# hasindu2008/sigtk

Hardware: NVIDIA B200
Metric: event_detection_throughput (higher is better)
Workload: dtype f64

## Files before the change

sigtk_b200/csrc/walk_core.cuh:

```cuda
#pragma once
#include <float.h>
#include <math.h>
#include <stdint.h>
#include <string.h>

#if defined(__CUDACC__)
#define SGW_HD __host__ __device__ __forceinline__
#else
#define SGW_HD inline
#endif

namespace sgpu {
namespace walk {

#if defined(__CUDA_ARCH__)
SGW_HD double dadd(double a, double b) { return __dadd_rn(a, b); }
SGW_HD double dsub(double a, double b) { return __dsub_rn(a, b); }
SGW_HD double dmul(double a, double b) { return __dmul_rn(a, b); }
SGW_HD double dfma(double a, double b, double c) { return __fma_rn(a, b, c); }
SGW_HD double ddiv(double a, double b) { return __ddiv_rn(a, b); }
SGW_HD double dsqrt(double a) { return __dsqrt_rn(a); }
SGW_HD float fadd(float a, float b) { return __fadd_rn(a, b); }
SGW_HD float fsub(float a, float b) { return __fsub_rn(a, b); }
SGW_HD float fmul(float a, float b) { return __fmul_rn(a, b); }
SGW_HD float ffma(float a, float b, float c) { return __fmaf_rn(a, b, c); }
SGW_HD float fdiv(float a, float b) { return __fdiv_rn(a, b); }
SGW_HD float d2f(double a) { return __double2float_rn(a); }
SGW_HD uint32_t d_hi(double a) { return (uint32_t)__double2hiint(a); }
SGW_HD uint32_t d_lo(double a) { return (uint32_t)__double2loint(a); }
SGW_HD uint32_t f_bits(float a) { return __float_as_uint(a); }
SGW_HD float bits_f(uint32_t b) { return __uint_as_float(b); }
SGW_HD float rsqrt_seed(float a) {
    float y;
    asm("rsqrt.approx.ftz.f32 %0, %1;" : "=f"(y) : "f"(a));
    return y;
}
SGW_HD double widen_pos(float a) {
    return __longlong_as_double((long long)((unsigned long long)__float_as_uint(a) * 0x20000000ull + 0x3800000000000000ull));
}
SGW_HD double widen_abs(float a) { return (double)fabsf(a); }
SGW_HD uint32_t shr_clamp(uint32_t x, int s) {
    uint32_t r;
    asm("shr.b32 %0, %1, %2;" : "=r"(r) : "r"(x), "r"(s));
    return r;
}
struct F2 { float lo, hi; };
SGW_HD F2 f2mul(F2 a, F2 b) {
    F2 r;
    asm("{\n\t.reg .b64 a, b, d;\n\tmov.b64 a, {%2, %3};\n\tmov.b64 b, {%4, %5};\n\tmul.rn.f32x2 d, a, b;\n\t"
        "mov.b64 {%0, %1}, d;\n\t}" : "=f"(r.lo), "=f"(r.hi) : "f"(a.lo), "f"(a.hi), "f"(b.lo), "f"(b.hi));
    return r;
}
SGW_HD F2 f2sq(F2 a) {
    F2 r;
    asm("{\n\t.reg .b64 a, d;\n\tmov.b64 a, {%2, %3};\n\tmul.rn.f32x2 d, a, a;\n\tmov.b64 {%0, %1}, d;\n\t}"
        : "=f"(r.lo), "=f"(r.hi) : "f"(a.lo), "f"(a.hi));
    return r;
}
SGW_HD F2 f2add(F2 a, F2 b) {
    F2 r;
    asm("{\n\t.reg .b64 a, b, d;\n\tmov.b64 a, {%2, %3};\n\tmov.b64 b, {%4, %5};\n\tadd.rn.f32x2 d, a, b;\n\t"
        "mov.b64 {%0, %1}, d;\n\t}" : "=f"(r.lo), "=f"(r.hi) : "f"(a.lo), "f"(a.hi), "f"(b.lo), "f"(b.hi));
    return r;
}
SGW_HD F2 f2sub(F2 a, F2 b) {
    F2 r;
    asm("{\n\t.reg .b64 a, b, d;\n\tmov.b64 a, {%2, %3};\n\tmov.b64 b, {%4, %5};\n\tsub.rn.f32x2 d, a, b;\n\t"
        "mov.b64 {%0, %1}, d;\n\t}" : "=f"(r.lo), "=f"(r.hi) : "f"(a.lo), "f"(a.hi), "f"(b.lo), "f"(b.hi));
    return r;
}
SGW_HD F2 f2fma(F2 a, F2 b, F2 c) {
    F2 r;
    asm("{\n\t.reg .b64 a, b, c, d;\n\tmov.b64 a, {%2, %3};\n\tmov.b64 b, {%4, %5};\n\tmov.b64 c, {%6, %7};\n\t"
        "fma.rn.f32x2 d, a, b, c;\n\tmov.b64 {%0, %1}, d;\n\t}"
        : "=f"(r.lo), "=f"(r.hi) : "f"(a.lo), "f"(a.hi), "f"(b.lo), "f"(b.hi), "f"(c.lo), "f"(c.hi));
    return r;
}
#else
SGW_HD double dadd(double a, double b) { return a + b; }
SGW_HD double dsub(double a, double b) { return a - b; }
SGW_HD double dmul(double a, double b) { return a * b; }
SGW_HD double dfma(double a, double b, double c) { return fma(a, b, c); }
SGW_HD double ddiv(double a, double b) { return a / b; }
SGW_HD double dsqrt(double a) { return sqrt(a); }
SGW_HD float fadd(float a, float b) { return a + b; }
SGW_HD float fsub(float a, float b) { return a - b; }
SGW_HD float fmul(float a, float b) { return a * b; }
SGW_HD float ffma(float a, float b, float c) { return fmaf(a, b, c); }
SGW_HD float fdiv(float a, float b) { return a / b; }
SGW_HD float d2f(double a) { return (float)a; }
SGW_HD uint32_t d_hi(double a) { uint64_t b; memcpy(&b, &a, 8); return (uint32_t)(b >> 32); }
SGW_HD uint32_t d_lo(double a) { uint64_t b; memcpy(&b, &a, 8); return (uint32_t)b; }
SGW_HD uint32_t f_bits(float a) { uint32_t b; memcpy(&b, &a, 4); return b; }
SGW_HD float bits_f(uint32_t b) { float a; memcpy(&a, &b, 4); return a; }
SGW_HD float rsqrt_seed(float a) { return (float)(1.0 / sqrt((double)a)); }
SGW_HD double widen_pos(float a) {
    uint32_t b; memcpy(&b, &a, 4);
    const uint64_t v = (uint64_t)b * 0x20000000ull + 0x3800000000000000ull;
    double r; memcpy(&r, &v, 8); return r;
}
SGW_HD double widen_abs(float a) { return (double)fabsf(a); }
SGW_HD uint32_t shr_clamp(uint32_t x, int s) { return (unsigned)s < 32u ? x >> s : 0u; }
struct F2 { float lo, hi; };
SGW_HD F2 f2mul(F2 a, F2 b) { F2 r; r.lo = a.lo * b.lo; r.hi = a.hi * b.hi; return r; }
SGW_HD F2 f2sq(F2 a) { F2 r; r.lo = a.lo * a.lo; r.hi = a.hi * a.hi; return r; }
SGW_HD F2 f2add(F2 a, F2 b) { F2 r; r.lo = a.lo + b.lo; r.hi = a.hi + b.hi; return r; }
SGW_HD F2 f2sub(F2 a, F2 b) { F2 r; r.lo = a.lo - b.lo; r.hi = a.hi - b.hi; return r; }
SGW_HD F2 f2fma(F2 a, F2 b, F2 c) { F2 r; r.lo = fmaf(a.lo, b.lo, c.lo); r.hi = fmaf(a.hi, b.hi, c.hi); return r; }
#endif

template <int RNA>
struct Cfg {
    static constexpr int w1 = RNA ? 7 : 3;
    static constexpr int w2 = 2 * w1;
    static constexpr int LAG = w2 - 1;
    static constexpr int R1 = RNA ? 8 : 4;
    static constexpr int R2 = RNA ? 16 : 8;
    static constexpr int U = RNA ? 16 : 8;
    static constexpr int FILL = 2;
    static_assert(FILL * U >= 2 * w2 - 1, "fill covers the look-back of the first step");
};
template <int RNA> SGW_HD float thr_short() { return RNA ? 2.5f : 1.4f; }
template <int RNA> SGW_HD float thr_long() { return 9.0f; }
template <int RNA> SGW_HD float peak_h() { return RNA ? 1.0f : 0.2f; }

template <int W>
SGW_HD double ddivw(double a) {
    constexpr double r = 1.0 / (double)W;
    const double q0 = dmul(a, r);
    const double e = dfma(-(double)W, q0, a);
    return dfma(e, r, q0);
}
template <int W>
SGW_HD float fdivw(float a) {
    constexpr float r = 1.0f / (float)W;
    const float q0 = fmul(a, r);
    const float e = ffma(-(float)W, q0, a);
    return ffma(e, r, q0);
}

template <int WA, int WB>
SGW_HD F2 fdivw2(F2 a) {
    const F2 r = {1.0f / (float)WA, 1.0f / (float)WB};
    const F2 nw = {-(float)WA, -(float)WB};
    const F2 q0 = f2mul(a, r);
    const F2 e = f2fma(nw, q0, a);
    return f2fma(e, r, q0);
}

SGW_HD float tail(float delta, float scaled, float scaled_half, float cv, bool& ok) {
    const double ch = widen_pos(scaled_half);
    const double y0 = widen_pos(rsqrt_seed(scaled));
    const double th = dmul(ch, y0);
    const double eh = dfma(-th, y0, 0.5);
    const double q0 = dmul(widen_abs(delta), y0);
    const double q = dfma(q0, eh, q0);
    ok = ok & ((d_lo(q) * 8u - ((0x10000000u - 1024u) << 3)) >= (2048u << 3)) & (cv >= 2.0e-29f);
    return d2f(q);
}

template <int W>
SGW_HD void window_terms(double D, double E, float& A, double& Lq, float& B, double& Vd, double& B2d) {
    A = d2f(ddivw<W>(D));
    const F2 de = {d2f(D), d2f(E)};
    const F2 bv = fdivw2<W, W>(de);
    Lq = dsub(ddivw<W>(E), widen_pos(fmul(A, A)));
    B = bv.lo;
    Vd = widen_pos(bv.hi);
    B2d = widen_pos(fmul(B, B));
}
template <int W>
SGW_HD void tstat_two(float A0, double L0, float B0, double V0, double B0sq, float A1, double L1, float B1, double V1,
                      double B1sq, float& t0, bool& ok0, float& t1, bool& ok1) {
    const double acc0 = dsub(dadd(L0, V0), B0sq);
    const double acc1 = dsub(dadd(L1, V1), B1sq);
    const F2 cv = {d2f(acc0), d2f(acc1)};
    const F2 sc = fdivw2<W, W>(cv);
    const F2 half = {0.5f, 0.5f};
    const F2 sh = f2mul(sc, half);
#if defined(WALK_X_NOTAIL)
    t0 = fmul(fsub(B0, A0), sc.lo); t1 = fmul(fsub(B1, A1), sh.hi);
#else
    t0 = tail(fsub(B0, A0), sc.lo, sh.lo, cv.lo, ok0);
    t1 = tail(fsub(B1, A1), sc.hi, sh.hi, cv.hi, ok1);
#endif
}

template <class Io>
SGW_HD float sample_pa(const Io& io, int i, int n, float off, float unit) {
    if (i < 0 || i >= n) return 0.0f;
    int v[4];
    io.load8(i & ~7, v);
    const int q = i & 7;
    const int word = q < 2 ? v[0] : q < 4 ? v[1] : q < 6 ? v[2] : v[3];
    const int raw = (q & 1) ? (word >> 16) : (int)(int16_t)(word & 0xffff);
    return fmul(fadd((float)raw, off), unit);
}
template <class Io>
SGW_HD void window_sums(const Io& io, int a, int w, int n, float off, float unit, double& S, double& Q) {
    S = 0.0; Q = 0.0;
    for (int i = a; i < a + w; i++) {
        const float x = sample_pa(io, i, n, off, unit);
        S = dadd(S, (double)x);
        Q = dadd(Q, (double)fmul(x, x));
    }
}
SGW_HD float tstat_from_sums(double sum1, double ssq1, double sum2d, double ssq2d, int w) {
    const float wf = (float)w;
    const float sum2 = d2f(sum2d), ssq2 = d2f(ssq2d);
    const float mean1 = d2f(ddiv(sum1, (double)wf));
    const float mean2 = fdiv(sum2, wf);
    double acc = ddiv(ssq1, (double)wf);
    acc = dsub(acc, (double)fmul(mean1, mean1));
    acc = dadd(acc, (double)fdiv(ssq2, wf));
    acc = dsub(acc, (double)fmul(mean2, mean2));
    const float cv = fmaxf(d2f(acc), FLT_MIN);
    const float delta = fsub(mean2, mean1);
    return d2f(ddiv(fabs((double)delta), dsqrt((double)fdiv(cv, wf))));
}
template <class Io>
SGW_HD float tstat_exact(const Io& io, int i, int w, int n, float off, float unit) {
    double sum1, ssq1, sum2d, ssq2d;
    window_sums(io, i - w, w, n, off, unit, sum1, ssq1);
    window_sums(io, i, w, n, off, unit, sum2d, ssq2d);
    return tstat_from_sums(sum1, ssq1, sum2d, ssq2d, w);
}
template <class Io>
struct SlidingT {
    double s1, q1, s2, q2;
    int at;
    SGW_HD SlidingT() : s1(0.0), q1(0.0), s2(0.0), q2(0.0), at(-1) {}
    SGW_HD float next(const Io& io, int i, int w, int n, float off, float unit) {
        if (!(i >= w && i + w <= n)) { at = -1; return 0.0f; }
        if (at != i - 1) {
            window_sums(io, i - w, w, n, off, unit, s1, q1);
            window_sums(io, i, w, n, off, unit, s2, q2);
        } else {
            const float xa = sample_pa(io, i - 1 - w, n, off, unit);
            const float xb = sample_pa(io, i - 1, n, off, unit);
            const float xc = sample_pa(io, i - 1 + w, n, off, unit);
            const double da = (double)xa, db = (double)xb, dc = (double)xc;
            const double qa = (double)fmul(xa, xa), qb = (double)fmul(xb, xb), qc = (double)fmul(xc, xc);
            s1 = dadd(dsub(s1, da), db); q1 = dadd(dsub(q1, qa), qb);
            s2 = dadd(dsub(s2, db), dc); q2 = dadd(dsub(q2, qb), qc);
        }
        at = i;
        return tstat_from_sums(s1, q1, s2, q2, w);
    }
};
constexpr int PS_NONE = 0x7fff0000;
constexpr int PS_OPEN = 0x40000000;
constexpr int LS_PRED = -0x40000000;
constexpr int LS_CONT = 0x7fffffff;
struct WalkDet {
    float s_pv; int s_ps;
    int l_start;
    bool l_hot;
};
SGW_HD void det_cold(WalkDet& d, int first_step) {
    d.s_pv = FLT_MAX; d.s_ps = PS_NONE;
    d.l_start = first_step; d.l_hot = false;
}

struct Canon { int v[8]; };
template <int RNA>
SGW_HD Canon canon_of(const WalkDet& d, int b) {
    Canon c;
    (void)b;
    c.v[0] = (int)f_bits(d.s_pv); c.v[1] = d.s_ps; c.v[2] = 0; c.v[3] = 0; c.v[4] = 0; c.v[5] = 0;
    c.v[6] = d.l_start; c.v[7] = 0;
    return c;
}

template <int RNA> struct PkCfg {
    static constexpr int LEAD = 32 - Cfg<RNA>::U;
#if defined(WALK_TEST_FAR)
    static constexpr int FAR = 0;
#else
    static constexpr int FAR = LEAD - (Cfg<RNA>::w1 / 2 + 1);
#endif
};
struct PeakAcc { uint32_t mk; int oldest; int jobs, job_ls, job_end; };
struct NoEmit { SGW_HD void operator()(int) const {} };

template <bool SHORT, int RNA, class E>
SGW_HD int det_one(float& pv, int& ps, int m, int u, float c, float thr, PeakAcc& acc, bool& big2, int& p2,
                   const E& on_emit) {
    constexpr int w = SHORT ? Cfg<RNA>::w1 : Cfg<RNA>::w2;
    const float h = peak_h<RNA>();
    const bool none = ps == PS_NONE;
    const float df = fsub(c, pv);
    const float pvm = none ? fminf(pv, c) : fmaxf(pv, c);
    const bool rise1 = none & (df > h);
    const bool gt2 = !none & (df > 0.0f);
    big2 = !none & (pvm > thr);
    const bool drop = big2 & (df < -h);
    p2 = gt2 ? ((ps & PS_OPEN) | u) : ps;
    const int p3 = drop ? (p2 & ~PS_OPEN) : p2;
    const int over = (u - (w / 2 + 1)) - p3;
    const bool emit = over >= 0;
    acc.mk |= shr_clamp(1u << (PkCfg<RNA>::LEAD + m - (w / 2 + 1)), over);
    if (emit) on_emit(p3);
    pv = (rise1 | emit) ? c : pvm;
    ps = emit ? PS_NONE : p3;
    ps = rise1 ? (u | PS_OPEN) : ps;
    return over;
}

struct DualDet {
    float s_pv; int s_ps;
    float l_pv; int l_ps; int l_mt;
};
SGW_HD void dual_cold(DualDet& d, int first_step) {
    d.s_pv = FLT_MAX; d.s_ps = PS_NONE;
    d.l_pv = FLT_MAX; d.l_ps = PS_NONE; d.l_mt = first_step - 1;
}
SGW_HD Canon dual_canon(const DualDet& d, int b) {
    Canon c;
    c.v[0] = (int)f_bits(d.s_pv); c.v[1] = d.s_ps; c.v[2] = (int)f_bits(d.l_pv); c.v[3] = d.l_ps;
    c.v[4] = d.l_mt >= b ? d.l_mt : -1;
    c.v[5] = 0; c.v[6] = 0; c.v[7] = 0;
    return c;
}
template <int RNA, class E>
SGW_HD void dual_step(DualDet& d, int u, float c1, float c2, const E& on_emit) {
    bool maskl, unused_b; int p2, unused_p;
    PeakAcc unused; unused.mk = 0u; unused.oldest = 0;
    det_one<true, RNA>(d.s_pv, d.s_ps, 0, u, c1, thr_short<RNA>(), unused, maskl, p2, on_emit);
    d.l_mt = maskl ? (p2 & ~PS_OPEN) + Cfg<RNA>::w1 : d.l_mt;
    d.l_ps = maskl ? PS_NONE : d.l_ps;
    d.l_pv = maskl ? FLT_MAX : d.l_pv;
    const float c2m = d.l_mt < u ? c2 : FLT_MAX;
    det_one<false, RNA>(d.l_pv, d.l_ps, 0, u, c2m, thr_long<RNA>(), unused, unused_b, unused_p, on_emit);
}

constexpr int ZMAX = 1023;
struct LongK {
    float c0;
    float ca;
    float cw;
    float h2;
    float t2w;
    float cB;
    float thr;
};
template <int RNA>
SGW_HD LongK long_consts(int c0, float off, float thr_long) {
    constexpr float w = (float)Cfg<RNA>::w2;
    const float u = 5.9604644775390625e-08f;
    LongK k;
    k.c0 = (float)c0;
    const float M = fmul(fadd(fabsf(fadd(k.c0, off)), (float)(ZMAX + 2)), 1.0001f);
    k.ca = fmul(fmul(8.0f * u * w, M), 1.0001f);
    k.cw = w * (1.0f + 0.000244140625f);
    k.thr = thr_long;
    const float thr2 = fmul(thr_long, thr_long);
    k.h2 = fmul(thr2, 0.5f);
    k.t2w = fmul(thr2, w);
    k.cB = fmul(fmul(fmul(thr2, 64.0f * u * w * w), fmul(M, M)), 1.0001f);
    return k;
}
SGW_HD bool long_candidate(float dS, float T, float Q, const LongK& k) {
    const float g = fadd(fabsf(dS), k.ca);
    const float sq = ffma(T, T, fmul(dS, dS));
    const float lhs = ffma(fmul(g, g), k.cw, ffma(sq, k.h2, k.cB));
    const float rhs = fmul(Q, k.t2w);
    return !(lhs < rhs);
}

constexpr int DIRTY_BLOCKS = 3;
static_assert(2 * Cfg<0>::w2 - 1 <= 2 * Cfg<0>::U + 0 && 2 * Cfg<1>::w2 - 1 <= 2 * Cfg<1>::U, "windows reach at most two blocks ahead");

template <int RNA>
struct Rings {
    using C = Cfg<RNA>;
    double P[C::R1], PQ[C::R1];
    float A1[C::R1];
    double L1[C::R1];
    float T1c[C::w1];
    static constexpr int ZH2 = 2 * C::w2 - C::U;
    float Z1[C::U], Z2[ZH2];
    float zdS, zT, zQ;
    SGW_HD void clear() {
#pragma unroll
        for (int k = 0; k < C::R1; k++) { P[k] = 0.0; PQ[k] = 0.0; A1[k] = 0.0f; L1[k] = 0.0; }
#pragma unroll
        for (int k = 0; k < C::w1; k++) T1c[k] = 0.0f;
#pragma unroll
        for (int k = 0; k < C::U; k++) Z1[k] = 0.0f;
#pragma unroll
        for (int k = 0; k < ZH2; k++) Z2[k] = 0.0f;
        zdS = 0.0f; zT = 0.0f; zQ = 0.0f;
    }
};

template <int RNA, bool DIRECT, class E, class Io>
SGW_HD void det_step(WalkDet& d, int m, int u, float c1, bool cand, bool rec, PeakAcc& acc, const E& on_emit, Io& io) {
    bool maskl; int p2;
    const int over = det_one<true, RNA>(d.s_pv, d.s_ps, m, u, c1, thr_short<RNA>(), acc, maskl, p2, on_emit);
    acc.oldest = acc.oldest > over ? acc.oldest : over;
    bool hot = d.l_hot;
    if (maskl & hot & rec) {
        if (DIRECT) io.job(d.l_start, u);
        else { acc.job_ls = d.l_start; acc.job_end = u; acc.jobs++; }
    }
    const int ls = (p2 & ~PS_OPEN) + Cfg<RNA>::w1 + 1;
    d.l_start = maskl ? (ls > u ? ls : u) : d.l_start;
    hot = (hot & !maskl) | ((u >= d.l_start) & cand);
    d.l_hot = hot;
}

template <int RNA> struct Redo { WalkDet d; PeakAcc acc; float t1c[Cfg<RNA>::w1]; };
template <int RNA, bool EDGE, class Io>
#if defined(__CUDACC__)
__host__ __device__ __noinline__
#else
inline
#endif
Redo<RNA> redo_block(Io& io, Redo<RNA> in, int tau0, int n, int sh, bool rec, float off, float unit, float thr_long) {
    using C = Cfg<RNA>;
    constexpr int w1 = C::w1, w2 = C::w2, U = C::U;
    (void)thr_long;
    float e1[U];
    SlidingT<Io> slide;
    for (int m = 0; m < U; m++) e1[m] = slide.next(io, tau0 + m - w1 + 1, w1, n, off, unit);
    Redo<RNA> r;
    r.d = in.d; r.acc.mk = 0u; r.acc.oldest = 0; r.acc.jobs = 0;
    const int u0 = tau0 - w2 + 1 + sh;
    for (int m = 0; m < U; m++) {
        const int j2 = tau0 + m - w2 + 1;
        const float c1 = m >= w1 ? e1[m - w1] : in.t1c[m];
        if (!EDGE || (j2 >= 1 && j2 < n)) {
            PeakAcc unused; unused.mk = 0u; unused.oldest = 0; unused.jobs = 0;
            det_step<RNA, true>(r.d, 0, u0 + m, c1, true, rec, unused, [&](int pos) { if (rec) io.peak(pos); }, io);
        }
    }
    for (int k = 0; k < w1; k++) r.t1c[k] = e1[U - w1 + k];
    return r;
}

template <int RNA, bool EDGE, class Io>
SGW_HD void walk_block(Rings<RNA>& g, WalkDet& d, const float (&x)[Cfg<RNA>::U], const float (&z)[Cfg<RNA>::U], int tau0,
                       int n, int sh, bool rec, bool live, bool live_t1, int dirty, int zdirty, float off, float unit,
                       const LongK& lk, Io& io) {
    using C = Cfg<RNA>;
    constexpr int w1 = C::w1, w2 = C::w2, M1 = C::R1 - 1, M2 = C::R2 - 1, U = C::U;
    float t1v[U];
    bool ok = true, ok_t1 = true;
    const WalkDet d0 = d;
    PeakAcc acc;
    acc.mk = 0u; acc.oldest = 0; acc.jobs = 0;
    const int u0 = tau0 - w2 + 1 + sh;
    float xq[U];
#pragma unroll
    for (int m = 0; m < U; m += 2) {
        const F2 p = {x[m], x[m + 1]};
        const F2 q = f2sq(p);
        xq[m] = q.lo; xq[m + 1] = q.hi;
    }
    float zdS = g.zdS, zT = g.zT, zQ = g.zQ;
#pragma unroll
    for (int m0 = 0; m0 < U; m0 += 2) {
        float a1[2], b1[2]; double l1[2], v1[2], b1sq[2];
        float al[2]; double ll[2];
#pragma unroll
        for (int h = 0; h < 2; h++) {
            const int m = m0 + h;
            const double xd = widen_pos(x[m]);
            const double qd = widen_pos(xq[m]);
            const double pn = dadd(g.P[m & M1], EDGE ? (x[m] > 0.0f ? xd : 0.0) : xd);
            const double pqn = dadd(g.PQ[m & M1], EDGE ? (x[m] > 0.0f ? qd : 0.0) : qd);
            g.P[(m + 1) & M1] = pn;
            g.PQ[(m + 1) & M1] = pqn;
            const int s1 = (m - w1 + 1) & M1;
            const int s1l = (m - 2 * w1 + 1) & M1;
            const double d1 = dsub(pn, g.P[s1]), e1 = dsub(pqn, g.PQ[s1]);
            window_terms<w1>(d1, e1, a1[h], l1[h], b1[h], v1[h], b1sq[h]);
            al[h] = g.A1[s1l]; ll[h] = g.L1[s1l];
        }
        bool k0 = true, k1 = true;
        tstat_two<w1>(al[0], ll[0], b1[0], v1[0], b1sq[0], al[1], ll[1], b1[1], v1[1], b1sq[1], t1v[m0], k0, t1v[m0 + 1], k1);
#pragma unroll
        for (int h = 0; h < 2; h++) {
            const int m = m0 + h;
            bool kh = h ? k1 : k0;
            const int j1 = tau0 + m - w1 + 1;
            if (EDGE) {
                const bool in1 = (j1 >= w1) & (j1 + w1 <= n);
                kh = kh | !in1;
                t1v[m] = in1 ? t1v[m] : 0.0f;
            }
            if (m >= U - w1) ok_t1 = ok_t1 & kh; else ok = ok & kh;
            const int s1 = (m - w1 + 1) & M1;
            g.A1[s1] = a1[h]; g.L1[s1] = l1[h];
        }
#pragma unroll
        for (int h = 0; h < 2; h++) {
            const int m = m0 + h;
            const float zn = z[m];
            const float zm = m >= w2 ? z[m >= w2 ? m - w2 : 0] : g.Z1[m < w2 ? m + U - w2 : 0];
            const float zo = m >= 2 * w2 - U ? g.Z1[m >= 2 * w2 - U ? m + U - 2 * w2 : 0] : g.Z2[m < 2 * w2 - U ? m : 0];
#if defined(WALK_X_NOCAND)
            zT = fadd(zT, zn); (void)zm; (void)zo;
            bool cand = false;
#else
            zT = fadd(zT, fsub(zn, zo));
            zQ = fadd(zQ, fsub(fmul(zn, zn), fmul(zo, zo)));
            zdS = fadd(fadd(zdS, fadd(zn, zo)), fmul(zm, -2.0f));
            bool cand = long_candidate(zdS, zT, zQ, lk);
#endif
            const int j2 = tau0 + m - w2 + 1;
            if (EDGE) cand = cand & (j2 >= w2) & (j2 + w2 <= n);
            cand = cand | (zdirty > 0);
            const float c1 = m >= w1 ? t1v[m >= w1 ? m - w1 : 0] : g.T1c[m < w1 ? m : 0];
#if defined(WALK_X_NODET)
            d.s_pv = fadd(d.s_pv, c1); d.l_hot = d.l_hot | cand;
#elif defined(WALK_X_NOLIFE)
            { bool mk_; int p2_; const int over_ = det_one<true, RNA>(d.s_pv, d.s_ps, m, u0 + m, c1, thr_short<RNA>(), acc, mk_, p2_, NoEmit());
              acc.oldest = acc.oldest > over_ ? acc.oldest : over_; d.l_hot = d.l_hot | (cand & mk_); d.l_start += p2_ & 1; }
#else
            if (!EDGE || (j2 >= 1 && j2 < n)) det_step<RNA, false>(d, m, u0 + m, c1, cand, rec, acc, NoEmit(), io);
#endif
        }
    }
    g.zdS = zdS; g.zT = zT; g.zQ = zQ;
#pragma unroll
    for (int k = 0; k < Rings<RNA>::ZH2; k++) g.Z2[k] = g.Z1[k + U - Rings<RNA>::ZH2];
#pragma unroll
    for (int k = 0; k < U; k++) g.Z1[k] = z[k];
#if defined(WALK_TEST_REDO)
    ok = ok & ((tau0 / U) % 3 != 0);
#endif
    if (dirty > 0) { ok = false; ok_t1 = false; }
    if ((!ok & live) | (!ok_t1 & live_t1) | (rec & ((acc.oldest > PkCfg<RNA>::FAR) | (acc.jobs > 1)))) {
        Redo<RNA> in;
        in.d = d0; in.acc = acc;
#pragma unroll
        for (int k = 0; k < w1; k++) in.t1c[k] = g.T1c[k];
        const Redo<RNA> r = redo_block<RNA, EDGE>(io, in, tau0, n, sh, rec, off, unit, lk.thr);
        d = r.d; acc = r.acc;
#pragma unroll
        for (int k = 0; k < w1; k++) t1v[U - w1 + k] = r.t1c[k];
    }
    if (rec && acc.mk) io.peaks32(u0 - PkCfg<RNA>::LEAD, acc.mk);
    if (acc.jobs == 1) io.job(acc.job_ls, acc.job_end);
#pragma unroll
    for (int k = 0; k < w1; k++) g.T1c[k] = t1v[U - w1 + k];
}

SGW_HD uint32_t n_chunks(uint32_t n, uint32_t L) { return (n + L - 1u) / L; }

SGW_HD void cvt8(const int (&v)[4], float off, float unit, float c0, float* x, float* z) {
    const F2 bias = {8421376.0f, 8421376.0f}, off2 = {off, off}, unit2 = {unit, unit}, c2 = {c0, c0};
#pragma unroll
    for (int k = 0; k < 4; k++) {
        const uint32_t w = (uint32_t)v[k] ^ 0x80008000u;
        F2 r;
        r.lo = bits_f(0x4b000000u | (w & 0xffffu));
        r.hi = bits_f(0x4b000000u | (w >> 16));
        r = f2sub(r, bias);
        const F2 zz = f2sub(r, c2);
        r = f2mul(f2add(r, off2), unit2);
        x[2 * k] = r.lo;
        x[2 * k + 1] = r.hi;
        z[2 * k] = zz.lo;
        z[2 * k + 1] = zz.hi;
    }
}
SGW_HD void cvt8(const int (&v)[4], float off, float unit, float* x) {
    const F2 bias = {8421376.0f, 8421376.0f}, off2 = {off, off}, unit2 = {unit, unit};
#pragma unroll
    for (int k = 0; k < 4; k++) {
        const uint32_t w = (uint32_t)v[k] ^ 0x80008000u;
        F2 r;
        r.lo = bits_f(0x4b000000u | (w & 0xffffu));
        r.hi = bits_f(0x4b000000u | (w >> 16));
        r = f2mul(f2add(f2sub(r, bias), off2), unit2);
        x[2 * k] = r.lo;
        x[2 * k + 1] = r.hi;
    }
}
#if defined(__CUDA_ARCH__)
SGW_HD uint32_t min_s16x2(uint32_t a, uint32_t b) { return __vmins2(a, b); }
SGW_HD uint32_t max_s16x2(uint32_t a, uint32_t b) { return __vmaxs2(a, b); }
#else
SGW_HD uint32_t min_s16x2(uint32_t a, uint32_t b) {
    const int16_t al = (int16_t)(a & 0xffff), ah = (int16_t)(a >> 16), bl = (int16_t)(b & 0xffff), bh = (int16_t)(b >> 16);
    return (uint32_t)(uint16_t)(al < bl ? al : bl) | ((uint32_t)(uint16_t)(ah < bh ? ah : bh) << 16);
}
SGW_HD uint32_t max_s16x2(uint32_t a, uint32_t b) {
    const int16_t al = (int16_t)(a & 0xffff), ah = (int16_t)(a >> 16), bl = (int16_t)(b & 0xffff), bh = (int16_t)(b >> 16);
    return (uint32_t)(uint16_t)(al > bl ? al : bl) | ((uint32_t)(uint16_t)(ah > bh ? ah : bh) << 16);
}
#endif

#if defined(__CUDA_ARCH__)
SGW_HD bool any_le_s16x2(uint32_t a, uint32_t b) { return __vcmples2(a, b) != 0u; }
#else
SGW_HD bool any_le_s16x2(uint32_t a, uint32_t b) {
    return (int16_t)(a & 0xffff) <= (int16_t)(b & 0xffff) || (int16_t)(a >> 16) <= (int16_t)(b >> 16);
}
#endif
constexpr int LOW_MARGIN = 64;
SGW_HD int low_threshold(float off, bool* can) {
    float tf = floorf(-off);
    tf = tf < -40000.0f ? -40000.0f : tf > 40000.0f ? 40000.0f : tf;
    int t = (int)tf;
    for (int k = 0; k < 4 && fadd((float)(t + 1), off) <= 0.0f; k++) t++;
    for (int k = 0; k < 4 && fadd((float)t, off) > 0.0f; k++) t--;
    t += LOW_MARGIN;
    *can = t >= -32768;
    return t > 32767 ? 32767 : t < -32768 ? -32768 : t;
}
SGW_HD uint32_t pack_s16x2(int t) { return ((uint32_t)t & 0xffffu) * 0x10001u; }
SGW_HD int s16_lo(uint32_t v) { return (int)(int16_t)(v & 0xffffu); }
SGW_HD int s16_hi(uint32_t v) { return (int)v >> 16; }

SGW_HD int pivot_of(int a, int b, int c) {
    const int lo = a < b ? a : b, hi = a < b ? b : a;
    return c < lo ? lo : c > hi ? hi : c;
}

template <class Io>
SGW_HD void zero_low8(Io& io, int t, const int (&v)[4], int low_t, float* x) {
    uint32_t lo = 0xffffffffu, hi = 0u;
#pragma unroll
    for (int q = 0; q < 8; q++) {
        const int raw = (q & 1) ? (v[q >> 1] >> 16) : (int)(int16_t)(v[q >> 1] & 0xffff);
        if (raw <= low_t) {
            const uint32_t a = f_bits(x[q]) & 0x7fffffffu;
            if (a != 0u) { lo = a < lo ? a : lo; hi = a > hi ? a : hi; }
            x[q] = 0.0f;
        }
    }
    io.low_samples(t, lo, hi);
}

struct BlockCvt {
    bool can_low, zlo_on, zhi_on, pa;
    int low_t;
    uint32_t low2, zlo2, zhi2;
};
SGW_HD BlockCvt block_cvt(float off, int c0, bool want_pa) {
    BlockCvt k;
    k.low_t = low_threshold(off, &k.can_low);
    k.low2 = pack_s16x2(k.low_t);
    k.zlo2 = pack_s16x2(c0 - ZMAX - 1 < -32768 ? -32768 : c0 - ZMAX - 1);
    k.zhi2 = pack_s16x2(c0 + ZMAX + 1 > 32767 ? 32767 : c0 + ZMAX + 1);
    k.zlo_on = c0 - ZMAX - 1 >= -32768; k.zhi_on = c0 + ZMAX + 1 <= 32767;
    k.pa = want_pa;
    return k;
}
template <class Io>
SGW_HD void cvt_group(Io& io, const BlockCvt& k, const LongK& lk, const int (&v)[4], int t8, bool own, float off, float unit,
                      float* x, float* z, uint32_t& bmin, uint32_t& bmax, int& dirty) {
    const uint32_t m8 = min_s16x2(min_s16x2((uint32_t)v[0], (uint32_t)v[1]), min_s16x2((uint32_t)v[2], (uint32_t)v[3]));
    bmin = min_s16x2(bmin, m8);
    bmax = max_s16x2(max_s16x2(bmax, (uint32_t)v[0]), max_s16x2((uint32_t)v[1], max_s16x2((uint32_t)v[2], (uint32_t)v[3])));
    cvt8(v, off, unit, lk.c0, x, z);
    if (k.pa && own) io.store_pa8(t8, x);
    if (k.can_low & any_le_s16x2(m8, k.low2)) {
        dirty = DIRTY_BLOCKS;
        zero_low8(io, t8, v, k.low_t, x);
    }
}
template <int U>
SGW_HD void clamp_far(const BlockCvt& k, uint32_t bmin, uint32_t bmax, float* z, int& zdirty) {
    if ((k.zlo_on & any_le_s16x2(bmin, k.zlo2)) | (k.zhi_on & any_le_s16x2(k.zhi2, bmax))) {
        zdirty = DIRTY_BLOCKS;
#pragma unroll
        for (int q = 0; q < U; q++)
            z[q] = z[q] > (float)(ZMAX + 1) ? (float)(ZMAX + 1) : z[q] < -(float)(ZMAX + 1) ? -(float)(ZMAX + 1) : z[q];
    }
}

#if !defined(WALK_PF_BLOCKS)
#define WALK_PF_BLOCKS 12
#endif

template <int RNA, class Io>
SGW_HD void walk_interior(Io& io, int n, float off, float unit, int sh, int L, int W, int k, float thr_long) {
    using C = Cfg<RNA>;
    constexpr int U = C::U;
    const int s0 = k * L, s1 = s0 + L;
    const int t_live = s0 - W;
    Rings<RNA> g;
    g.clear();
    WalkDet d;
    det_cold(d, 0);
    float x[U], z[U];
    int v[4];
    uint32_t vmin = 0x7fff7fffu, vmax = 0x80008000u;
    int dirty = 0, zdirty = 0;
    int vn[U / 8][4];
#pragma unroll
    for (int h = 0; h < U / 8; h++) io.load8(t_live - C::FILL * U + 8 * h, vn[h]);
    const int c0 = pivot_of(s16_lo((uint32_t)vn[0][0]), s16_hi((uint32_t)vn[0][0]), s16_lo((uint32_t)vn[0][1]));
    const LongK lk = long_consts<RNA>(c0, off, thr_long);
    const BlockCvt bc = block_cvt(off, c0, io.want_pa());
#pragma unroll 1
    for (int tau = t_live - C::FILL * U; tau < s1; tau += U) {
        const bool own = tau >= s0;
        if (tau == t_live) det_cold(d, t_live - C::LAG + sh);
        if (tau == s0) {
            io.put_begin(canon_of<RNA>(d, s0 - C::LAG + sh));
            d.l_start = LS_PRED; d.l_hot = false;
        }
        const int tn = tau + U < s1 ? tau + U : tau;
        io.prefetch(tau + WALK_PF_BLOCKS * U < s1 ? tau + WALK_PF_BLOCKS * U : tau);
        uint32_t bmin = 0x7fff7fffu, bmax = 0x80008000u;
#pragma unroll
        for (int h = 0; h < U / 8; h++) {
#pragma unroll
            for (int q = 0; q < 4; q++) v[q] = vn[h][q];
            io.load8(tn + 8 * h, vn[h]);
            cvt_group(io, bc, lk, v, tau + 8 * h, own, off, unit, x + 8 * h, z + 8 * h, bmin, bmax, dirty);
        }
        vmin = min_s16x2(vmin, bmin);
        vmax = max_s16x2(vmax, bmax);
        clamp_far<U>(bc, bmin, bmax, z, zdirty);
        walk_block<RNA, false>(g, d, x, z, tau, n, sh, own, tau >= t_live, tau >= t_live - U, dirty, zdirty, off, unit, lk, io);
        dirty = dirty > 0 ? dirty - 1 : 0;
        zdirty = zdirty > 0 ? zdirty - 1 : 0;
    }
    if (d.l_hot) io.job(d.l_start, LS_CONT);
    io.put_end(canon_of<RNA>(d, s1 - C::LAG + sh));
    const int rmin0 = s16_lo(vmin), rmin1 = s16_hi(vmin);
    const int rmax0 = s16_lo(vmax), rmax1 = s16_hi(vmax);
    io.witness(rmin0 < rmin1 ? rmin0 : rmin1, rmax0 > rmax1 ? rmax0 : rmax1, bc.can_low ? bc.low_t : -32769);
}

#if defined(__CUDACC__)
#define SGW_PHASE __host__ __device__ __noinline__
#else
#define SGW_PHASE inline
#endif
template <int RNA>
struct EdgeCtx {
    Rings<RNA> g;
    WalkDet d;
    int rmin, rmax, dirty, zdirty;
    int n, sh, s0, s1, t_live, last, low_t, c0;
    float off, unit;
    bool pa;
    LongK lk;
    BlockCvt bc;
};
template <int RNA, class Io>
SGW_HD void edge_block_begin(Io& io, EdgeCtx<RNA>& e, int tau) {
    using C = Cfg<RNA>;
    if (e.last && tau == e.t_live) det_cold(e.d, e.t_live - C::LAG + e.sh);
    if (e.last && tau == e.s0) {
        io.put_begin(canon_of<RNA>(e.d, e.s0 - C::LAG + e.sh));
        e.d.l_start = LS_PRED; e.d.l_hot = false;
    }
}
template <int RNA, class Io>
SGW_PHASE void edge_inner(Io& io, EdgeCtx<RNA>& ec, int tau_from, int tau_to) {
    using C = Cfg<RNA>;
    constexpr int U = C::U;
    const int turns = io.warp_max(tau_to > tau_from ? (tau_to - tau_from) / U : 0);
    EdgeCtx<RNA> e = ec;
    float x[U], z[U];
    int vn[U / 8][4];
    if (tau_from < tau_to) {
#pragma unroll
        for (int h = 0; h < U / 8; h++) io.load8(tau_from + 8 * h, vn[h]);
    }
    int tau = tau_from;
#pragma unroll 1
    for (int turn = 0; turn < turns; turn++, tau += U) {
        if (tau >= tau_to) continue;
        const bool own = tau >= e.s0;
        edge_block_begin<RNA>(io, e, tau);
        const int tn = tau + U < tau_to ? tau + U : tau;
        io.prefetch(tau + WALK_PF_BLOCKS * U < tau_to ? tau + WALK_PF_BLOCKS * U : tau);
        uint32_t bmin = 0x7fff7fffu, bmax = 0x80008000u;
#pragma unroll
        for (int h = 0; h < U / 8; h++) {
            int v[4];
#pragma unroll
            for (int q = 0; q < 4; q++) v[q] = vn[h][q];
            io.load8(tn + 8 * h, vn[h]);
            cvt_group(io, e.bc, e.lk, v, tau + 8 * h, own, e.off, e.unit, x + 8 * h, z + 8 * h, bmin, bmax, e.dirty);
        }
        if (own) {
            const int b0 = s16_lo(bmin), b1 = s16_hi(bmin), c0x = s16_lo(bmax), c1x = s16_hi(bmax);
            e.rmin = b0 < e.rmin ? b0 : e.rmin; e.rmin = b1 < e.rmin ? b1 : e.rmin;
            e.rmax = c0x > e.rmax ? c0x : e.rmax; e.rmax = c1x > e.rmax ? c1x : e.rmax;
        }
        clamp_far<U>(e.bc, bmin, bmax, z, e.zdirty);
        walk_block<RNA, false>(e.g, e.d, x, z, tau, e.n, e.sh, own, tau >= e.t_live, tau >= e.t_live - U, e.dirty, e.zdirty,
                               e.off, e.unit, e.lk, io);
        e.dirty = e.dirty > 0 ? e.dirty - 1 : 0;
        e.zdirty = e.zdirty > 0 ? e.zdirty - 1 : 0;
    }
    ec = e;
}
template <int RNA, class Io>
SGW_PHASE void edge_checked(Io& io, EdgeCtx<RNA>& ec, int tau_from, int tau_to) {
    using C = Cfg<RNA>;
    constexpr int U = C::U;
    const int turns = io.warp_max(tau_to > tau_from ? (tau_to - tau_from) / U : 0);
    EdgeCtx<RNA> e = ec;
    float x[U], z[U];
    const int n = e.n, c0 = e.c0, low_t = e.low_t;
    int tau = tau_from;
#pragma unroll 1
    for (int turn = 0; turn < turns; turn++, tau += U) {
        if (tau >= tau_to) continue;
        const bool own = tau >= e.s0;
        edge_block_begin<RNA>(io, e, tau);
#pragma unroll
        for (int h = 0; h < U / 8; h++) {
            const int t8 = tau + 8 * h;
            int v[4] = {0, 0, 0, 0};
            if (t8 < n) io.load8(t8, v);
            float y[8], zy[8];
            cvt8(v, e.off, e.unit, e.lk.c0, y, zy);
#pragma unroll
            for (int q = 0; q < 8; q++) {
                const bool in = t8 + q < n;
                const int raw = (q & 1) ? (v[q >> 1] >> 16) : (int)(int16_t)(v[q >> 1] & 0xffff);
                const bool low = in & (raw <= low_t);
                x[8 * h + q] = (in & !low) ? y[q] : 0.0f;
                const bool zbad = in & ((raw - c0 > ZMAX) | (c0 - raw > ZMAX));
                z[8 * h + q] = !in ? 0.0f : !zbad ? zy[q] : raw > c0 ? (float)(ZMAX + 1) : -(float)(ZMAX + 1);
                if (zbad) e.zdirty = DIRTY_BLOCKS;
                if (low) {
                    e.dirty = DIRTY_BLOCKS;
                    const uint32_t a = f_bits(y[q]) & 0x7fffffffu;
                    io.low_samples(t8 + q, a != 0u ? a : 0xffffffffu, a);
                }
                if (own && in && t8 + q < e.s1) {
                    e.rmin = raw < e.rmin ? raw : e.rmin;
                    e.rmax = raw > e.rmax ? raw : e.rmax;
                    if (e.pa) io.store_pa1(t8 + q, y[q]);
                }
            }
        }
        walk_block<RNA, true>(e.g, e.d, x, z, tau, n, e.sh, own, tau >= e.t_live, tau >= e.t_live - U, e.dirty, e.zdirty,
                              e.off, e.unit, e.lk, io);
        e.dirty = e.dirty > 0 ? e.dirty - 1 : 0;
        e.zdirty = e.zdirty > 0 ? e.zdirty - 1 : 0;
    }
    ec = e;
}

template <int RNA, class Io>
SGW_HD void walk_edge(Io& io, int n, float off, float unit, int sh, int L, int W, int last, float thr_long) {
    using C = Cfg<RNA>;
    constexpr int U = C::U;
    const uint32_t nch = n_chunks((uint32_t)n, (uint32_t)L);
    const bool none = nch == 0u || (last && nch < 2u);
    EdgeCtx<RNA> e;
    e.n = n; e.sh = sh; e.off = off; e.unit = unit; e.last = last;
    e.s0 = last ? (int)(nch - 1u) * L : 0;
    const bool to_end = last || nch == 1u;
    e.s1 = to_end ? n : L;
    e.t_live = last ? e.s0 - W : 0;
    const int step_end = to_end ? n : e.s1 - C::LAG;
    e.g.clear();
    det_cold(e.d, sh + 1);
    e.rmin = 32767; e.rmax = -32768;
    bool can_low;
    const int low_t0 = low_threshold(off, &can_low);
    e.low_t = can_low ? low_t0 : -32769;
    e.dirty = 0; e.zdirty = 0;
    e.pa = io.want_pa();
    const int t_first = last ? e.t_live - C::FILL * U : 0;
    e.c0 = 0;
    if (!none) {
        int v0[4] = {0, 0, 0, 0};
        io.load8(t_first, v0);
        const int a = s16_lo((uint32_t)v0[0]), b = t_first + 1 < n ? s16_hi((uint32_t)v0[0]) : a;
        e.c0 = pivot_of(a, b, t_first + 2 < n ? s16_lo((uint32_t)v0[1]) : a);
    }
    e.lk = long_consts<RNA>(e.c0, off, thr_long);
    e.bc = block_cvt(off, e.c0, e.pa);
    constexpr int INNER_MIN = (2 * C::w2 - 1 + U - 1) / U * U;
    const int tau_end = none ? t_first : (step_end + C::LAG + U - 1) / U * U;
    int in0 = t_first > INNER_MIN ? t_first : INNER_MIN;
    in0 = in0 < tau_end ? in0 : tau_end;
    int in1 = n / U * U;
    in1 = in1 < tau_end ? in1 : tau_end;
    in1 = in1 > in0 ? in1 : in0;
    edge_checked<RNA>(io, e, t_first, in0);
    edge_inner<RNA>(io, e, in0, in1);
    edge_checked<RNA>(io, e, in1, tau_end);
    if (none) return;
    if (to_end) {
        if (e.d.l_hot) io.job(e.d.l_start, n + sh);
    } else {
        if (e.d.l_hot) io.job(e.d.l_start, LS_CONT);
        io.put_end(canon_of<RNA>(e.d, e.s1 - C::LAG + sh));
    }
    if (!last) io.peak(sh);
    if (e.rmin <= e.rmax) io.witness(e.rmin, e.rmax, e.low_t);
}

template <int RNA, class Jo>
SGW_HD void long_job(Jo& io, int n, int sh, float off, float unit, int L, int k, int l_start, int end, float thr_long) {
    using C = Cfg<RNA>;
    constexpr int w1 = C::w1, w2 = C::w2;
    for (int kk = k - 1; l_start == LS_PRED && kk >= 0; kk--) l_start = io.end_lstart(kk);
    if (l_start == LS_PRED) return;
    const int stop = n + sh;
    const int own_end = end == LS_CONT ? (k + 1) * L - C::LAG + sh : (end < stop ? end : stop);
    float pv = FLT_MAX; int ps = PS_NONE;
    PeakAcc unused; unused.mk = 0u; unused.oldest = 0;
    bool b2; int p2;
    SlidingT<Jo> slide;
    int u = l_start;
    for (; u + 4 <= own_end; u += 4) {
        float t[4];
#pragma unroll
        for (int q = 0; q < 4; q++) t[q] = slide.next(io, u + q - sh, w2, n, off, unit);
#pragma unroll
        for (int q = 0; q < 4; q++)
            det_one<false, RNA>(pv, ps, 0, u + q, t[q], thr_long, unused, b2, p2, [&](int pos) { io.peak(pos); });
    }
    for (; u < own_end; u++)
        det_one<false, RNA>(pv, ps, 0, u, slide.next(io, u - sh, w2, n, off, unit), thr_long, unused, b2, p2,
                            [&](int pos) { io.peak(pos); });
    if (end != LS_CONT) return;
    float spv; int sps;
    io.end_short(k, &spv, &sps);
    u = own_end;
    SlidingT<Jo> slide1;
    for (; u < stop; u++) {
        const float t1 = slide1.next(io, u - sh, w1, n, off, unit);
        const float t2 = slide.next(io, u - sh, w2, n, off, unit);
        det_one<true, RNA>(spv, sps, 0, u, t1, thr_short<RNA>(), unused, b2, p2, NoEmit());
        if (b2) return;
        det_one<false, RNA>(pv, ps, 0, u, t2, thr_long, unused, b2, p2, [&](int pos) { io.peak(pos); });
    }
}

}
}
```

Baseline: 127.1.

## Rework long-window candidate test into pairwise FMA form with tighter clamp range

Rewrites the long-window candidate filter as a single sign test of a precomputed quadratic form (k1*dS^2 + T^2 - 2w*Q + K0), evaluated for two consecutive samples at once with paired float ops and shared running-sum updates. It also lowers the clamp range for RNA so the long-window sums stay exact in float, and drops an unused parameter from redo_block. The goal is fewer float instructions per sample in the hot walk loop. The risks are a more conservative bound that flags more candidates and more clamping for RNA inputs, which sends more work to the slow path.

```diff
diff --git a/sigtk_b200/csrc/walk_core.cuh b/sigtk_b200/csrc/walk_core.cuh
--- a/sigtk_b200/csrc/walk_core.cuh
+++ b/sigtk_b200/csrc/walk_core.cuh
@@ -119,6 +119,9 @@
     static constexpr int U = RNA ? 16 : 8;
     static constexpr int FILL = 2;
     static_assert(FILL * U >= 2 * w2 - 1, "fill covers the look-back of the first step");
+    static constexpr int ZFAR = RNA ? 773 : 1023;
+    static_assert(2 * w2 * (ZFAR + 1) * (ZFAR + 1) <= (1 << 24), "long-window sums exact in float");
+    static_assert(w2 % 2 == 0 && U % 2 == 0 && (2 * w2 - U) % 2 == 0, "the long window's pairs sit at even indices");
 };
 template <int RNA> SGW_HD float thr_short() { return RNA ? 2.5f : 1.4f; }
 template <int RNA> SGW_HD float thr_long() { return 9.0f; }
@@ -337,35 +340,40 @@
 constexpr int ZMAX = 1023;
 struct LongK {
     float c0;
-    float ca;
-    float cw;
-    float h2;
-    float t2w;
-    float cB;
+    float k1;
+    float K0;
+    float n2w;
     float thr;
 };
 template <int RNA>
 SGW_HD LongK long_consts(int c0, float off, float thr_long) {
     constexpr float w = (float)Cfg<RNA>::w2;
+    constexpr float cw = 2.0f * w * (1.0f + 0.000244140625f);
     const float u = 5.9604644775390625e-08f;
     LongK k;
     k.c0 = (float)c0;
+    k.thr = thr_long;
+    k.n2w = -2.0f * w;
     const float M = fmul(fadd(fabsf(fadd(k.c0, off)), (float)(ZMAX + 2)), 1.0001f);
-    k.ca = fmul(fmul(8.0f * u * w, M), 1.0001f);
-    k.cw = w * (1.0f + 0.000244140625f);
-    k.thr = thr_long;
+    const float a = fmul(fmul(8.0f * u * w, M), 1.0001f);
     const float thr2 = fmul(thr_long, thr_long);
-    k.h2 = fmul(thr2, 0.5f);
-    k.t2w = fmul(thr2, w);
-    k.cB = fmul(fmul(fmul(thr2, 64.0f * u * w * w), fmul(M, M)), 1.0001f);
+    k.k1 = fmul(fadd(1.0f, fmul(fdiv(fmul(cw, 1.0009765625f), thr2), 1.0001f)), 1.0001f);
+    k.K0 = fmul(fadd(fdiv(fmul(fmul(cw, 1025.0f), fmul(a, a)), thr2), fmul(128.0f * u * w * w, fmul(M, M))), 1.0001f);
+    const bool in_range = (thr_long >= 9.5367431640625e-07f) & (M <= 1.099511627776e12f);
+    k.k1 = in_range ? k.k1 : 0.0f;
+    k.K0 = in_range ? k.K0 : INFINITY;
     return k;
 }
+SGW_HD F2 long_test(F2 dS, F2 T, F2 Q, const LongK& k, float n2w_) {
+    const F2 n2w = {n2w_, n2w_}, k1 = {k.k1, k.k1}, K0 = {k.K0, k.K0};
+    const F2 r1 = f2fma(Q, n2w, K0);
+    const F2 r2 = f2fma(f2mul(k1, dS), dS, r1);
+    return f2fma(T, T, r2);
+}
+SGW_HD bool long_cold(float r) { return (f_bits(r) >> 31) != 0u; }
 SGW_HD bool long_candidate(float dS, float T, float Q, const LongK& k) {
-    const float g = fadd(fabsf(dS), k.ca);
-    const float sq = ffma(T, T, fmul(dS, dS));
-    const float lhs = ffma(fmul(g, g), k.cw, ffma(sq, k.h2, k.cB));
-    const float rhs = fmul(Q, k.t2w);
-    return !(lhs < rhs);
+    const F2 dS2 = {dS, dS}, T2 = {T, T}, Q2 = {Q, Q};
+    return !long_cold(long_test(dS2, T2, Q2, k, k.n2w).lo);
 }
 
 constexpr int DIRTY_BLOCKS = 3;
@@ -417,10 +425,9 @@
 #else
 inline
 #endif
-Redo<RNA> redo_block(Io& io, Redo<RNA> in, int tau0, int n, int sh, bool rec, float off, float unit, float thr_long) {
+Redo<RNA> redo_block(Io& io, Redo<RNA> in, int tau0, int n, int sh, bool rec, float off, float unit) {
     using C = Cfg<RNA>;
     constexpr int w1 = C::w1, w2 = C::w2, U = C::U;
-    (void)thr_long;
     float e1[U];
     SlidingT<Io> slide;
     for (int m = 0; m < U; m++) e1[m] = slide.next(io, tau0 + m - w1 + 1, w1, n, off, unit);
@@ -494,31 +501,43 @@
             const int s1 = (m - w1 + 1) & M1;
             g.A1[s1] = a1[h]; g.L1[s1] = l1[h];
         }
+        uint32_t lr[2];
+        {
+            const int b1 = m0 >= w2 ? m0 - w2 : m0 + U - w2, b2 = m0 >= 2 * w2 - U ? m0 + U - 2 * w2 : m0;
+            const F2 zn = {z[m0], z[m0 + 1]};
+            const F2 zm = m0 >= w2 ? F2{z[b1], z[b1 + 1]} : F2{g.Z1[b1], g.Z1[b1 + 1]};
+            const F2 zo = m0 >= 2 * w2 - U ? F2{g.Z1[b2], g.Z1[b2 + 1]} : F2{g.Z2[b2], g.Z2[b2 + 1]};
+#if defined(WALK_X_NOCAND)
+            zT = fadd(zT, fadd(zn.lo, zn.hi)); (void)zm; (void)zo;
+            lr[0] = 0xffffffffu; lr[1] = 0xffffffffu;
+#else
+            const F2 sp = f2add(zn, zo);
+            const F2 dz = f2sub(zn, zo);
+            const F2 m2 = {-2.0f, -2.0f};
+            const F2 ds = f2fma(zm, m2, sp);
+            F2 S, T, Q;
+            T.lo = fadd(zT, dz.lo);
+            T.hi = fadd(T.lo, dz.hi);
+            S.lo = fadd(zdS, ds.lo);
+            S.hi = fadd(S.lo, ds.hi);
+            Q.lo = ffma(dz.lo, sp.lo, zQ);
+            Q.hi = ffma(dz.hi, sp.hi, Q.lo);
+            zT = T.hi; zdS = S.hi; zQ = Q.hi;
+            const F2 r = long_test(S, T, Q, lk, -2.0f * w2);
+            lr[0] = f_bits(r.lo); lr[1] = f_bits(r.hi);
+#endif
+        }
 #pragma unroll
         for (int h = 0; h < 2; h++) {
             const int m = m0 + h;
-            const float zn = z[m];
-            const float zm = m >= w2 ? z[m >= w2 ? m - w2 : 0] : g.Z1[m < w2 ? m + U - w2 : 0];
-            const float zo = m >= 2 * w2 - U ? g.Z1[m >= 2 * w2 - U ? m + U - 2 * w2 : 0] : g.Z2[m < 2 * w2 - U ? m : 0];
-#if defined(WALK_X_NOCAND)
-            zT = fadd(zT, zn); (void)zm; (void)zo;
-            bool cand = false;
+            const int j2 = tau0 + m - w2 + 1;
+            const float c1 = m >= w1 ? t1v[m >= w1 ? m - w1 : 0] : g.T1c[m < w1 ? m : 0];
+#if defined(WALK_X_NODET)
+            d.s_pv = fadd(d.s_pv, c1); d.l_hot = d.l_hot | ((lr[h] >> 31) == 0u);
 #else
-            zT = fadd(zT, fsub(zn, zo));
-            zQ = fadd(zQ, fsub(fmul(zn, zn), fmul(zo, zo)));
-            zdS = fadd(fadd(zdS, fadd(zn, zo)), fmul(zm, -2.0f));
-            bool cand = long_candidate(zdS, zT, zQ, lk);
-#endif
-            const int j2 = tau0 + m - w2 + 1;
+            bool cand = (lr[h] >> 31) == 0u;
             if (EDGE) cand = cand & (j2 >= w2) & (j2 + w2 <= n);
             cand = cand | (zdirty > 0);
-            const float c1 = m >= w1 ? t1v[m >= w1 ? m - w1 : 0] : g.T1c[m < w1 ? m : 0];
-#if defined(WALK_X_NODET)
-            d.s_pv = fadd(d.s_pv, c1); d.l_hot = d.l_hot | cand;
-#elif defined(WALK_X_NOLIFE)
-            { bool mk_; int p2_; const int over_ = det_one<true, RNA>(d.s_pv, d.s_ps, m, u0 + m, c1, thr_short<RNA>(), acc, mk_, p2_, NoEmit());
-              acc.oldest = acc.oldest > over_ ? acc.oldest : over_; d.l_hot = d.l_hot | (cand & mk_); d.l_start += p2_ & 1; }
-#else
             if (!EDGE || (j2 >= 1 && j2 < n)) det_step<RNA, false>(d, m, u0 + m, c1, cand, rec, acc, NoEmit(), io);
 #endif
         }
@@ -537,7 +556,7 @@
         in.d = d0; in.acc = acc;
 #pragma unroll
         for (int k = 0; k < w1; k++) in.t1c[k] = g.T1c[k];
-        const Redo<RNA> r = redo_block<RNA, EDGE>(io, in, tau0, n, sh, rec, off, unit, lk.thr);
+        const Redo<RNA> r = redo_block<RNA, EDGE>(io, in, tau0, n, sh, rec, off, unit);
         d = r.d; acc = r.acc;
 #pragma unroll
         for (int k = 0; k < w1; k++) t1v[U - w1 + k] = r.t1c[k];
@@ -641,13 +660,15 @@
     int low_t;
     uint32_t low2, zlo2, zhi2;
 };
+template <int RNA>
 SGW_HD BlockCvt block_cvt(float off, int c0, bool want_pa) {
+    constexpr int ZFAR = Cfg<RNA>::ZFAR;
     BlockCvt k;
     k.low_t = low_threshold(off, &k.can_low);
     k.low2 = pack_s16x2(k.low_t);
-    k.zlo2 = pack_s16x2(c0 - ZMAX - 1 < -32768 ? -32768 : c0 - ZMAX - 1);
-    k.zhi2 = pack_s16x2(c0 + ZMAX + 1 > 32767 ? 32767 : c0 + ZMAX + 1);
-    k.zlo_on = c0 - ZMAX - 1 >= -32768; k.zhi_on = c0 + ZMAX + 1 <= 32767;
+    k.zlo2 = pack_s16x2(c0 - ZFAR - 1 < -32768 ? -32768 : c0 - ZFAR - 1);
+    k.zhi2 = pack_s16x2(c0 + ZFAR + 1 > 32767 ? 32767 : c0 + ZFAR + 1);
+    k.zlo_on = c0 - ZFAR - 1 >= -32768; k.zhi_on = c0 + ZFAR + 1 <= 32767;
     k.pa = want_pa;
     return k;
 }
@@ -664,13 +685,14 @@
         zero_low8(io, t8, v, k.low_t, x);
     }
 }
-template <int U>
+template <int RNA>
 SGW_HD void clamp_far(const BlockCvt& k, uint32_t bmin, uint32_t bmax, float* z, int& zdirty) {
+    constexpr int ZFAR = Cfg<RNA>::ZFAR, U = Cfg<RNA>::U;
     if ((k.zlo_on & any_le_s16x2(bmin, k.zlo2)) | (k.zhi_on & any_le_s16x2(k.zhi2, bmax))) {
         zdirty = DIRTY_BLOCKS;
 #pragma unroll
         for (int q = 0; q < U; q++)
-            z[q] = z[q] > (float)(ZMAX + 1) ? (float)(ZMAX + 1) : z[q] < -(float)(ZMAX + 1) ? -(float)(ZMAX + 1) : z[q];
+            z[q] = z[q] > (float)(ZFAR + 1) ? (float)(ZFAR + 1) : z[q] < -(float)(ZFAR + 1) ? -(float)(ZFAR + 1) : z[q];
     }
 }
 
@@ -697,7 +719,7 @@
     for (int h = 0; h < U / 8; h++) io.load8(t_live - C::FILL * U + 8 * h, vn[h]);
     const int c0 = pivot_of(s16_lo((uint32_t)vn[0][0]), s16_hi((uint32_t)vn[0][0]), s16_lo((uint32_t)vn[0][1]));
     const LongK lk = long_consts<RNA>(c0, off, thr_long);
-    const BlockCvt bc = block_cvt(off, c0, io.want_pa());
+    const BlockCvt bc = block_cvt<RNA>(off, c0, io.want_pa());
 #pragma unroll 1
     for (int tau = t_live - C::FILL * U; tau < s1; tau += U) {
         const bool own = tau >= s0;
@@ -718,7 +740,7 @@
         }
         vmin = min_s16x2(vmin, bmin);
         vmax = max_s16x2(vmax, bmax);
-        clamp_far<U>(bc, bmin, bmax, z, zdirty);
+        clamp_far<RNA>(bc, bmin, bmax, z, zdirty);
         walk_block<RNA, false>(g, d, x, z, tau, n, sh, own, tau >= t_live, tau >= t_live - U, dirty, zdirty, off, unit, lk, io);
         dirty = dirty > 0 ? dirty - 1 : 0;
         zdirty = zdirty > 0 ? zdirty - 1 : 0;
@@ -789,7 +811,7 @@
             e.rmin = b0 < e.rmin ? b0 : e.rmin; e.rmin = b1 < e.rmin ? b1 : e.rmin;
             e.rmax = c0x > e.rmax ? c0x : e.rmax; e.rmax = c1x > e.rmax ? c1x : e.rmax;
         }
-        clamp_far<U>(e.bc, bmin, bmax, z, e.zdirty);
+        clamp_far<RNA>(e.bc, bmin, bmax, z, e.zdirty);
         walk_block<RNA, false>(e.g, e.d, x, z, tau, e.n, e.sh, own, tau >= e.t_live, tau >= e.t_live - U, e.dirty, e.zdirty,
                                e.off, e.unit, e.lk, io);
         e.dirty = e.dirty > 0 ? e.dirty - 1 : 0;
@@ -804,6 +826,7 @@
     const int turns = io.warp_max(tau_to > tau_from ? (tau_to - tau_from) / U : 0);
     EdgeCtx<RNA> e = ec;
     float x[U], z[U];
+    constexpr int ZFAR = C::ZFAR;
     const int n = e.n, c0 = e.c0, low_t = e.low_t;
     int tau = tau_from;
 #pragma unroll 1
@@ -824,8 +847,8 @@
                 const int raw = (q & 1) ? (v[q >> 1] >> 16) : (int)(int16_t)(v[q >> 1] & 0xffff);
                 const bool low = in & (raw <= low_t);
                 x[8 * h + q] = (in & !low) ? y[q] : 0.0f;
-                const bool zbad = in & ((raw - c0 > ZMAX) | (c0 - raw > ZMAX));
-                z[8 * h + q] = !in ? 0.0f : !zbad ? zy[q] : raw > c0 ? (float)(ZMAX + 1) : -(float)(ZMAX + 1);
+                const bool zbad = in & ((raw - c0 > ZFAR) | (c0 - raw > ZFAR));
+                z[8 * h + q] = !in ? 0.0f : !zbad ? zy[q] : raw > c0 ? (float)(ZFAR + 1) : -(float)(ZFAR + 1);
                 if (zbad) e.zdirty = DIRTY_BLOCKS;
                 if (low) {
                     e.dirty = DIRTY_BLOCKS;
@@ -877,7 +900,7 @@
         e.c0 = pivot_of(a, b, t_first + 2 < n ? s16_lo((uint32_t)v0[1]) : a);
     }
     e.lk = long_consts<RNA>(e.c0, off, thr_long);
-    e.bc = block_cvt(off, e.c0, e.pa);
+    e.bc = block_cvt<RNA>(off, e.c0, e.pa);
     constexpr int INNER_MIN = (2 * C::w2 - 1 + U - 1) / U * U;
     const int tau_end = none ? t_first : (step_end + C::LAG + U - 1) / U * U;
     int in0 = t_first > INNER_MIN ? t_first : INNER_MIN;
```

Measured after the change: 130.6 (median of 6 runs). 1.03x the previous value.
